# darnstrom/LinearMPC.jl

Hardware: AMD Instinct MI355X
Metric: condensed-MPC QP solves/sec (batch 1e6 params), pendulum Nc=5 (higher is better)
Workload: dtype f64; 1 GPU; pendulum: inverted pendulum on cart, 4 states / 1 input, Np=50 Nc=5 (n=5 vars, 5 two-sided input bounds, theta=[x;r;u_prev] nth=7), 1000000 parameter points per GPU, cold start, first move u0 returned; batch_per_gpu=1000000, kernel=fast<5>|screen+lane<5>, batches_in_flight=3, rotating_batches=6

## Files before the change

### linearmpc.jl_amd/csrc/lmpc_fast_inst.hip

```cpp
#include <hip/hip_runtime.h>

#include <cstdio>
#include <cstdlib>
#include <vector>

#include "lmpc_internal.hpp"
#include "lmpc_fast_kernel.hpp"

namespace lmpc {

bool fast_covers(const lmpc_handle *h) {
    const HostPack &P = h->P;
    constexpr int kmax = LMPC_FAST_KMAX;
    return h->fastPath && !h->useWave && h->laneN >= 2 && h->laneN <= 5 && P.n == h->laneN && P.m == P.n && P.ms == P.m &&
           P.nth >= 1 && P.nth <= (h->laneN == 5 ? 8 : 16) && h->L.eq_mask == 0ull && h->L.imm_mask == 0ull && P.nsoft == 0 && !h->bnb &&
           h->S.iter_limit > kmax + 1 && h->S.cycle_tol >= kmax + 1;
}

template <int NTHMAX, int NT, int N, bool GATHER>
static int launch_fast_t(lmpc_handle *h, int64_t nprob, const double *theta, double *x, int32_t *flag, int32_t *iters,
                         uint64_t *active, hipStream_t st) {
    const int nstr = h->fastNstr >= 1 && h->fastNstr <= 4 ? h->fastNstr : 3;
    const long long ntiles = (nprob + 63) / 64;
    long long slots = (long long)h->numCU * LMPC_FAST_WAVES;
    long long Rl = (ntiles + slots - 1) / slots;
    if (Rl < 8) Rl = 8;
    if (h->fastTiles > 0) Rl = h->fastTiles;
    if (Rl > kFastMaxTiles) Rl = kFastMaxTiles;
    if (Rl > ntiles) Rl = ntiles > 0 ? ntiles : 1;
    const int R = (int)Rl;
    const unsigned grid = (unsigned)((ntiles + R - 1) / R);
    int D = GATHER ? 0 : (h->fastDyn >= 0 ? h->fastDyn : 0);
    if (R < 12 || nprob >= (int64_t)0x7fffff00 || D >= R) D = 0;
    const int Rs = R - D, Dcap = 3 * D, Rq = D ? Rs + Dcap + 1 : R;
    int dk = GATHER ? 0 : (h->fastDma >= 0 ? h->fastDma : (nstr <= 3 ? LMPC_FAST_DMA_DEPTH : 0));
    if (dk == 1 || dk > 3) dk = dk == 1 ? 0 : 3;
    if (nprob * (int64_t)NT * 8 < 16) dk = 0;
    if ((reinterpret_cast<uintptr_t>(theta) & 15u) != 0 || (fast_tile_bytes(NT) & 15u) != 0) dk = 0;
    const size_t lds = dk ? fast_lds_bytes_dma(N, Rq, NTHMAX, NT, nstr, dk) : fast_lds_bytes(N, Rq, NTHMAX);
    int32_t *ctrNow = nullptr, *ctrNext = nullptr;
    if (D) {
        if (!h->dFastCtr) {
            HIP_TRY(h, hipMalloc(&h->dFastCtr, sizeof(int32_t) * 2 * kFastCtrs * 32));
            HIP_TRY(h, hipMemsetAsync(h->dFastCtr, 0, sizeof(int32_t) * 2 * kFastCtrs * 32, st));
        }
        ctrNow = h->dFastCtr + (size_t)h->fastCtrSet * kFastCtrs * 32;
        ctrNext = h->dFastCtr + (size_t)(h->fastCtrSet ^ 1) * kFastCtrs * 32;
        h->fastCtrSet ^= 1;
    }
    auto kern = fast_kernel<NTHMAX, NT, N, GATHER>;
    if (lds > 48 * 1024)
        HIP_TRY(h, hipFuncSetAttribute((const void *)kern, hipFuncAttributeMaxDynamicSharedMemorySize, (int)lds));
    if (!h->dFastErr) {
#ifdef LMPC_FAST_TRACE
        const size_t eb = 64 + sizeof(long long) * 8 * 4 * 65536;
        HIP_TRY(h, hipMalloc(&h->dFastErr, eb));
        HIP_TRY(h, hipMemsetAsync(h->dFastErr, 0, eb, st));
#else
        int32_t *hp = nullptr;
        HIP_TRY(h, hipHostMalloc(reinterpret_cast<void **>(&hp), 64, hipHostMallocMapped));
        *hp = 0;
        h->hFastErr = hp;
        HIP_TRY(h, hipHostGetDevicePointer(reinterpret_cast<void **>(&h->dFastErr), hp, 0));
#endif
    }
    hipLaunchKernelGGL(kern, dim3(grid), dim3(256), lds, st, h->L, h->dC, theta, x, flag, iters,
                       active, (long long)nprob, Rq, nstr, h->dFastErr, h->fastSpinLimit > 0 ? h->fastSpinLimit - 1 : kFastSpinLimit,
                       dk, Rs, Dcap, ctrNow, ctrNext);
    HIP_TRY(h, hipGetLastError());
#ifdef LMPC_FAST_TRACE
    if (const char *f = std::getenv("LMPC_FAST_TRACE_FILE")) {
        std::vector<long long> tr((size_t)grid * 4 * 8);
        if (hipStreamSynchronize(st) == hipSuccess &&
            hipMemcpy(tr.data(), reinterpret_cast<char *>(h->dFastErr) + 64, sizeof(long long) * tr.size(), hipMemcpyDeviceToHost) == hipSuccess) {
            if (FILE *fp = std::fopen(f, "wb")) { std::fwrite(tr.data(), sizeof(long long), tr.size(), fp); std::fclose(fp); }
        }
    }
#endif
    return LMPC_OK;
}

template <int NTHMAX, int NT, int N>
static int launch_fast_multi_t(lmpc_handle *h, int nb, int64_t nprob, const double *const *theta, double *const *x,
                               int32_t *const *flag, hipStream_t st) {
    const int nstr = h->fastNstr >= 1 && h->fastNstr <= 4 ? h->fastNstr : 3;
    const long long ntiles = (nprob + 63) / 64;
    long long slots = (long long)h->numCU * LMPC_FAST_WAVES;
    long long Rl = (ntiles + slots - 1) / slots;
    if (Rl < 8) Rl = 8;
    if (h->fastTiles > 0) Rl = h->fastTiles;
    if (Rl > kFastMaxTiles) Rl = kFastMaxTiles;
    if (Rl > ntiles) Rl = ntiles > 0 ? ntiles : 1;
    const int R = (int)Rl;
    const unsigned grid = (unsigned)((ntiles + R - 1) / R);
    int dk = h->fastDma >= 0 ? h->fastDma : (nstr <= 3 ? LMPC_FAST_DMA_DEPTH : 0);
    if (dk == 1 || dk > 3) dk = dk == 1 ? 0 : 3;
    if (nprob * (int64_t)NT * 8 < 16 || (fast_tile_bytes(NT) & 15u) != 0) dk = 0;
    FastBatches B{};
    for (int b = 0; b < nb; b++) {
        B.theta[b] = theta[b]; B.x[b] = x[b]; B.flag[b] = flag[b];
        if ((reinterpret_cast<uintptr_t>(theta[b]) & 15u) != 0) dk = 0;
    }
    const size_t lds = dk ? fast_lds_bytes_dma(N, R, NTHMAX, NT, nstr, dk) : fast_lds_bytes(N, R, NTHMAX);
    auto kern = fast_kernel_multi<NTHMAX, NT, N>;
    if (lds > 48 * 1024)
        HIP_TRY(h, hipFuncSetAttribute((const void *)kern, hipFuncAttributeMaxDynamicSharedMemorySize, (int)lds));
    if (!h->dFastErr) {
        int32_t *hp = nullptr;
        HIP_TRY(h, hipHostMalloc(reinterpret_cast<void **>(&hp), 64, hipHostMallocMapped));
        *hp = 0;
        h->hFastErr = hp;
        HIP_TRY(h, hipHostGetDevicePointer(reinterpret_cast<void **>(&h->dFastErr), hp, 0));
    }
    hipLaunchKernelGGL(kern, dim3(grid, (unsigned)nb), dim3(256), lds, st, h->L, h->dC, B, (long long)nprob, R, nstr, h->dFastErr,
                       h->fastSpinLimit > 0 ? h->fastSpinLimit - 1 : kFastSpinLimit, dk);
    HIP_TRY(h, hipGetLastError());
    return LMPC_OK;
}

int launch_fast_multi(lmpc_handle *h, int nb, int64_t nprob, const double *const *theta, double *const *x, int32_t *const *flag,
                      hipStream_t st) {
    if (nb < 1 || nb > kFastMaxBatches) return LMPC_ERR_UNSUPPORTED;
#ifdef LMPC_FAST_TRACE
    return LMPC_ERR_UNSUPPORTED;
#else
#define LMPC_FM(NM, NT)                                                                                     \
    switch (h->laneN) {                                                                                     \
        case 2: return launch_fast_multi_t<NM, NT, 2>(h, nb, nprob, theta, x, flag, st);                    \
        case 3: return launch_fast_multi_t<NM, NT, 3>(h, nb, nprob, theta, x, flag, st);                    \
        case 4: return launch_fast_multi_t<NM, NT, 4>(h, nb, nprob, theta, x, flag, st);                    \
        case 5: if constexpr (NT <= 8) return launch_fast_multi_t<NM, NT, 5>(h, nb, nprob, theta, x, flag, st); break; \
        default: break;                                                                                     \
    }                                                                                                       \
    break;
    switch (h->P.nth) {
#ifdef LMPC_FAST_ONLY_PENDULUM
        case 7: if (h->laneN == 5) return launch_fast_multi_t<8, 7, 5>(h, nb, nprob, theta, x, flag, st); break;
#else
        case 1: LMPC_FM(8, 1)   case 2: LMPC_FM(8, 2)   case 3: LMPC_FM(8, 3)   case 4: LMPC_FM(8, 4)
        case 5: LMPC_FM(8, 5)   case 6: LMPC_FM(8, 6)   case 7: LMPC_FM(8, 7)   case 8: LMPC_FM(8, 8)
        case 9: LMPC_FM(16, 9)  case 10: LMPC_FM(16, 10) case 11: LMPC_FM(16, 11) case 12: LMPC_FM(16, 12)
        case 13: LMPC_FM(16, 13) case 14: LMPC_FM(16, 14) case 15: LMPC_FM(16, 15) case 16: LMPC_FM(16, 16)
#endif
        default: break;
    }
#undef LMPC_FM
    return LMPC_ERR_UNSUPPORTED;
#endif
}

int check_fast_err(lmpc_handle *h) {
    if (!h->hFastErr) return LMPC_OK;
    const int32_t e = *h->hFastErr;
    if (e == 0) return LMPC_OK;
    *h->hFastErr = 0;
    return fail(h, LMPC_ERR_HIP, "lmpc: the one-launch kernel gave up a bounded wait (code " + std::to_string(e) +
                                 ") in an earlier call on this handle: problems it had queued keep exit flag -8 "
                                 "(LMPC_EXIT_UNFINISHED), their x is not a solution");
}

void fast_preload(lmpc_handle *h) {
    hipFuncAttributes fa;
    (void)hipFuncGetAttributes(&fa, (const void *)fast_kernel<8, 7, 5, false>);
    if (h && !h->dFastCtr && hipMalloc(&h->dFastCtr, sizeof(int32_t) * 2 * kFastCtrs * 32) == hipSuccess)
        (void)hipMemset(h->dFastCtr, 0, sizeof(int32_t) * 2 * kFastCtrs * 32);
#ifndef LMPC_FAST_TRACE
    if (h && !h->dFastErr) {
        int32_t *hp = nullptr;
        if (hipHostMalloc(reinterpret_cast<void **>(&hp), 64, hipHostMallocMapped) == hipSuccess) {
            *hp = 0;
            if (hipHostGetDevicePointer(reinterpret_cast<void **>(&h->dFastErr), hp, 0) == hipSuccess) h->hFastErr = hp;
            else { (void)hipHostFree(hp); h->dFastErr = nullptr; }
        }
    }
#endif
    (void)hipGetLastError();
}

int launch_fast(lmpc_handle *h, int64_t nprob, const double *theta, double *x, int32_t *flag, int32_t *iters,
                uint64_t *active, hipStream_t st) {
    const bool gather = h->L.gat.state != nullptr;
#define LMPC_FN(NM, NT)                                                                                               \
    switch (h->laneN) {                                                                                               \
        case 2: return gather ? launch_fast_t<NM, NT, 2, true>(h, nprob, theta, x, flag, iters, active, st) : launch_fast_t<NM, NT, 2, false>(h, nprob, theta, x, flag, iters, active, st);    \
        case 3: return gather ? launch_fast_t<NM, NT, 3, true>(h, nprob, theta, x, flag, iters, active, st) : launch_fast_t<NM, NT, 3, false>(h, nprob, theta, x, flag, iters, active, st);    \
        case 4: return gather ? launch_fast_t<NM, NT, 4, true>(h, nprob, theta, x, flag, iters, active, st) : launch_fast_t<NM, NT, 4, false>(h, nprob, theta, x, flag, iters, active, st);    \
        case 5: if constexpr (NT <= 8) return gather ? launch_fast_t<NM, NT, 5, true>(h, nprob, theta, x, flag, iters, active, st) : launch_fast_t<NM, NT, 5, false>(h, nprob, theta, x, flag, iters, active, st); break; \
        default: break;                                                                                               \
    }                                                                                                                 \
    break;
    switch (h->P.nth) {
#ifdef LMPC_FAST_ONLY_PENDULUM
        case 7: if (h->laneN == 5) return gather ? launch_fast_t<8, 7, 5, true>(h, nprob, theta, x, flag, iters, active, st) : launch_fast_t<8, 7, 5, false>(h, nprob, theta, x, flag, iters, active, st); break;
#else
        case 1: LMPC_FN(8, 1)   case 2: LMPC_FN(8, 2)   case 3: LMPC_FN(8, 3)   case 4: LMPC_FN(8, 4)
        case 5: LMPC_FN(8, 5)   case 6: LMPC_FN(8, 6)   case 7: LMPC_FN(8, 7)   case 8: LMPC_FN(8, 8)
        case 9: LMPC_FN(16, 9)  case 10: LMPC_FN(16, 10) case 11: LMPC_FN(16, 11) case 12: LMPC_FN(16, 12)
        case 13: LMPC_FN(16, 13) case 14: LMPC_FN(16, 14) case 15: LMPC_FN(16, 15) case 16: LMPC_FN(16, 16)
#endif
        default: break;
    }
#undef LMPC_FN
    return fail(h, LMPC_ERR_UNSUPPORTED, "lmpc: no fast-kernel instantiation");
}

}
```

### linearmpc.jl_amd/csrc/lmpc_fast_kernel.hpp

```cpp
#pragma once

#include <hip/hip_runtime.h>
#include <stdint.h>

#include "lmpc_lane_kernel.hpp"
#include "lmpc_tiers.hpp"

namespace lmpc {

#ifndef LMPC_FAST_WAVES
#define LMPC_FAST_WAVES 3
#endif
constexpr int kFastSpinLimit = 1 << 22;
constexpr int kFastCtrs = 16;
constexpr int kFastMaxTiles = 96;
#ifndef LMPC_FAST_AHEAD
#define LMPC_FAST_AHEAD 1
#endif
constexpr int kFastAhead = LMPC_FAST_AHEAD;

#ifndef LMPC_FAST_DMA_POLICY
#define LMPC_FAST_DMA_POLICY " nt"
#endif
__device__ __forceinline__ void fast_dma16(const void *gsrc, unsigned lds_dst) {
    unsigned keep;
    asm volatile("s_mov_b32 %0, m0\n\ts_mov_b32 m0, %2\n\ts_nop 0\n\tglobal_load_lds_dwordx4 %1, off" LMPC_FAST_DMA_POLICY
                 "\n\ts_mov_b32 m0, %0"
                 : "=&s"(keep) : "v"(gsrc), "s"(lds_dst) : "memory");
}
#ifndef LMPC_FAST_DMA_DEPTH
#define LMPC_FAST_DMA_DEPTH 2
#endif
__host__ __device__ constexpr size_t fast_tile_bytes(int NT) { return (size_t)64 * NT * sizeof(double); }

__device__ __forceinline__ int lds_load(const int *p) {
    return __hip_atomic_load(p, __ATOMIC_RELAXED, __HIP_MEMORY_SCOPE_WORKGROUP);
}

__host__ __device__ constexpr int fast_scr_doubles(int N, int NTHMAX) { return (N * NTHMAX + 2 * N + NTHMAX + 1 + 1) & ~1; }
#ifndef LMPC_FAST_PAY
#define LMPC_FAST_PAY 256
#endif
constexpr int kFastPay = LMPC_FAST_PAY;
__host__ __device__ constexpr size_t fast_lds_bytes(int N, int R, int NTHMAX) {
    return sizeof(double) * (size_t)(((N * N + N * (N + 1) / 2 + 2 * N + 1) & ~1) + 4 * N * 64 + fast_scr_doubles(N, NTHMAX) +
                                     (size_t)kFastPay * (N + 1)) +
           sizeof(int32_t) * ((size_t)R * 64 + 4);
}
__host__ __device__ constexpr size_t fast_lds_bytes_dma(int N, int R, int NTHMAX, int NT, int nstr, int dk) {
    return fast_lds_bytes(N, R, NTHMAX) + (size_t)dk * nstr * fast_tile_bytes(NT);
}

template <int NTHMAX, int NT, int N, bool GATHER = false>
__device__ __forceinline__ void fast_body(
    const PackLayout &P, const double *__restrict__ C, const double *__restrict__ theta,
    double *__restrict__ X, int32_t *__restrict__ exitflag, int32_t *__restrict__ iters,
    uint64_t *__restrict__ active, long long nprob, int R, int nstr, int32_t *__restrict__ errflag, int spinLimit,
    int dk, int Rs, int Dcap, int32_t *__restrict__ tctr, int32_t *__restrict__ tctr_next) {
    constexpr int KMAX = LMPC_FAST_KMAX < N ? LMPC_FAST_KMAX : N;
    constexpr int nconst = N * N + N * (N + 1) / 2 + 2 * N;
    extern __shared__ __align__(16) double lds[];
    double *sconst = lds;
    double *sBall = sconst + ((nconst + 1) & ~1);
    double *sScr = sBall + 4 * N * 64;
    double *sPay = sScr + fast_scr_doubles(N, NTHMAX);
    int32_t *ring = reinterpret_cast<int32_t *>(sPay + (size_t)kFastPay * (N + 1));
    int *ctrl = reinterpret_cast<int *>(ring + R * 64);
    const int tid = threadIdx.x, lane = tid & 63;
    const int wv = __builtin_amdgcn_readfirstlane(tid >> 6);
    const int nth = P.nth;
    for (int i = tid; i < nconst; i += 256) sconst[i] = C[P.oM + i];
    for (int i = tid; i < N * NTHMAX; i += 256) sScr[i] = C[P.oDthP + i];
    if (tid < 2 * N) sScr[N * NTHMAX + tid] = C[P.oBnd + tid];
    if (tid < NTHMAX) sScr[N * NTHMAX + 2 * N + tid] = C[P.oXthP + tid];
    if (tid == 0) sScr[N * NTHMAX + 2 * N + NTHMAX] = C[P.ox0];
    for (int i = tid; i < R * 64; i += 256) ring[i] = -1;
    if (tid < 4) ctrl[tid] = 0;
    __syncthreads();
    const double *sM = sconst, *sG = sM + N * N, *sdu = sG + N * (N + 1) / 2, *sdl = sdu + N;
    double *sB = sBall + wv * N * 64;
    const double ntol = -P.primal_tol;
    const long long ntiles = (nprob + 63) / 64;
#ifdef LMPC_FAST_TRACE
    long long *trc = reinterpret_cast<long long *>(errflag + 16) + ((long long)blockIdx.x * 4 + wv) * 8;
    int npass = 0;
#define LMPC_TRC(i) do { if (lane == 0) trc[i] = (long long)wall_clock64(); } while (0)
#else
#define LMPC_TRC(i) do { } while (0)
#endif
    LMPC_TRC(0);
    const bool dyn = tctr != nullptr;
    const long long nstat = dyn ? ((long long)gridDim.x * Rs < ntiles ? (long long)gridDim.x * Rs : ntiles) : ntiles;
    if (dyn && blockIdx.x == 0 && tid < kFastCtrs) tctr_next[tid * 32] = 0;
    const long long t0 = (long long)blockIdx.x * (dyn ? Rs : R);
    const long long t1 = t0 + (dyn ? Rs : R) < nstat ? t0 + (dyn ? Rs : R) : nstat;
    const long long base0 = dyn ? 0 : t0 * 64;

    auto load_record = [&](long long pid, double *dst) {
        const long long pc = pid < nprob ? pid : nprob - 1;
        if constexpr (GATHER) {
            const GatherArgs &Ga = P.gat;
            const int o1 = Ga.nx, o2 = o1 + Ga.nr, o3 = o2 + Ga.nd, o4 = o3 + Ga.nup;
#pragma unroll
            for (int t = 0; t < NT; t++) {
                double v = 0.0;
                if (t < o1) v = Ga.state[pc * Ga.nx + t];
                else if (t < o2) { if (Ga.reference) v = Ga.reference[pc * Ga.nr + (t - o1)]; }
                else if (t < o3) { if (Ga.disturbance) v = Ga.disturbance[pc * Ga.nd + (t - o2)]; }
                else if (t < o4) { if (Ga.control) v = Ga.control[pc * Ga.ncontrol + (t - o3)]; }
                else { if (Ga.parameter) v = Ga.parameter[pc * Ga.np + (t - o4)]; }
                dst[t] = v;
            }
        } else {
            const double *src = theta + pc * nth;
#pragma unroll
            for (int t = 0; t < NT; t++) dst[t] = src[t];
        }
    };
    auto write_x = [&](long long pid, const double (&th)[NT], const double (&u)[N], bool with_u) {
        const double *xk = C + P.oXthP;
        for (int k = 0; k < P.nout; k++, xk += NTHMAX) {
            double sh = C[P.ox0 + k];
#pragma unroll
            for (int t = 0; t < NT; t++) sh = __builtin_fma(xk[t], th[t], sh);
            double xs = 0.0;
            if (with_u) {
#pragma unroll
                for (int c = 0; c < N; c++) xs = __builtin_fma(C[P.oRout + k * N + c], u[c], xs);
            }
            X[pid * P.nout + k] = xs + sh;
        }
    };

    const int role = (wv + (int)(blockIdx.x & 3)) & 3;
    if (role < nstr) {
        double buf[kFastAhead][NT];
        auto process = [&](long long tile, const double (&th)[NT], bool live) {
            const long long pid = tile * 64 + lane;
            const bool valid = live && pid < nprob;
            typedef const double __attribute__((address_space(3))) *lds_cdp;
            unsigned scr_off = (unsigned)(size_t)(lds_cdp)sScr;
            asm volatile("" : "+v"(scr_off));
            const lds_cdp scr = (lds_cdp)(size_t)scr_off;
            bool hard = false;
            typedef double v2d __attribute__((ext_vector_type(2)));
            typedef const v2d __attribute__((address_space(3))) *lds_c2p;
            const lds_c2p c2 = (lds_c2p)(size_t)scr_off;
            static_assert(NTHMAX % 2 == 0, "rows of pairs");
            double bq[N];
#pragma unroll
            for (int j = 0; j < N; j++) {
                double row[NTHMAX];
#pragma unroll
                for (int q = 0; q < (NT + 1) / 2; q++) {
                    const v2d v = c2[j * (NTHMAX / 2) + q];
                    row[2 * q] = v.x; row[2 * q + 1] = v.y;
                }
                double acc = 0.0;
#pragma unroll
                for (int t = 0; t < NT; t++) acc = __builtin_fma(row[t], th[t], acc);
                bq[j] = acc;
                const v2d bb = c2[N * (NTHMAX / 2) + j];
                const double vu = (bb.x + acc) - 0.0;
                const double vl = -((bb.y + acc) - 0.0);
                hard = hard | (vu < ntol) | (vl < ntol);
            }
            hard = hard & valid;
            double sh = scr[N * NTHMAX + 2 * N + NTHMAX];
            {
                double row[NTHMAX];
#pragma unroll
                for (int q = 0; q < (NT + 1) / 2; q++) {
                    const v2d v = c2[(N * NTHMAX + 2 * N) / 2 + q];
                    row[2 * q] = v.x; row[2 * q + 1] = v.y;
                }
#pragma unroll
                for (int t = 0; t < NT; t++) sh = __builtin_fma(row[t], th[t], sh);
            }
            const unsigned long long mask = __ballot(hard);
#ifdef LMPC_FAST_NT_STORES
            if (valid) __builtin_nontemporal_store(hard ? EXIT_UNFINISHED : EXIT_OPTIMAL, &exitflag[pid]);
#else
            if (valid) exitflag[pid] = hard ? EXIT_UNFINISHED : EXIT_OPTIMAL;
#endif
            if (mask != 0ull) {
                int base = 0;
                if (lane == 0) base = __hip_atomic_fetch_add(&ctrl[0], __popcll(mask), __ATOMIC_RELAXED, __HIP_MEMORY_SCOPE_WORKGROUP);
                base = __shfl(base, 0);
                if (hard) {
                    const int pos = base + __popcll(mask & ((1ull << lane) - 1ull));
                    if (pos < kFastPay) {
                        double *pay = sPay + pos * (N + 1);
#pragma unroll
                        for (int j = 0; j < N; j++) pay[j] = bq[j];
                        pay[N] = sh;
                    }
                    __hip_atomic_store(&ring[pos], (int32_t)(pid - base0), __ATOMIC_RELEASE, __HIP_MEMORY_SCOPE_WORKGROUP);
                }
            }
            if (valid && !hard) {
                if (P.nout == 1) {
#ifdef LMPC_FAST_NT_STORES
                    __builtin_nontemporal_store(0.0 + sh, &X[pid]);
#else
                    X[pid] = 0.0 + sh;
#endif
                } else {
                    double u0[N];
#pragma unroll
                    for (int c = 0; c < N; c++) u0[c] = 0.0;
                    write_x(pid, th, u0, false);
                }
                if (iters) iters[pid] = 1;
                if (active) active[pid * P.words] = 0ull;
            }
        };
#ifdef LMPC_FAST_CONTIG
        const long long per = (R + nstr - 1) / nstr;
        const long long s0 = t0 + role * per, s1 = s0 + per < t1 ? s0 + per : t1;
        for (long long base = s0; base < s1; base += kFastAhead) {
#pragma unroll
            for (int d = 0; d < kFastAhead; d++) {
                const long long tl = base + d;
                load_record((tl < s1 ? tl : base) * 64 + lane, buf[d]);
            }
#pragma unroll
            for (int d = 0; d < kFastAhead; d++) {
                const long long tl = base + d;
                process(tl < s1 ? tl : base, buf[d], tl < s1);
            }
        }
#elif defined(LMPC_FAST_PP)
        {
            double bufB[NT];
            long long tile = t0 + role;
            if (tile < t1) {
                load_record(tile * 64 + lane, buf[0]);
                for (;;) {
                    long long nxt = tile + nstr < t1 ? tile + nstr : tile;
                    load_record(nxt * 64 + lane, bufB);
                    process(tile, buf[0], true);
                    if (tile + nstr >= t1) break;
                    tile += nstr;
                    nxt = tile + nstr < t1 ? tile + nstr : tile;
                    load_record(nxt * 64 + lane, buf[0]);
                    process(tile, bufB, true);
                    if (tile + nstr >= t1) break;
                    tile += nstr;
                }
            }
        }
#else
        if (!GATHER && dk >= 2) {
            constexpr unsigned TB = (unsigned)fast_tile_bytes(NT);
            constexpr int PIECES = (int)((TB + 1023) / 1024);
            constexpr unsigned LASTB = TB - (PIECES - 1) * 1024u;
            typedef const double __attribute__((address_space(3))) *lds_cdp;
            char *dring = reinterpret_cast<char *>(ctrl + 4) + (size_t)role * dk * TB;
            const unsigned dbase = (unsigned)(size_t)(lds_cdp) reinterpret_cast<double *>(dring);
            const char *tbytes = reinterpret_cast<const char *>(theta);
            const long long tfull = nprob / 64;
            const long long te = t1 < tfull ? t1 : tfull;
            auto issue = [&](long long tile, int slot) {
                const char *src = tbytes + tile * (long long)TB + lane * 16;
#pragma unroll
                for (int p = 0; p < PIECES; p++) {
                    const unsigned dst = __builtin_amdgcn_readfirstlane(dbase + (unsigned)slot * TB + (unsigned)p * 1024u);
                    if (p + 1 < PIECES || LASTB == 1024u || lane * 16 < (int)LASTB) fast_dma16(src + p * 1024, dst);
                }
            };
            int cc = (int)((blockIdx.x * (unsigned)nstr + (unsigned)role) & (kFastCtrs - 1));
            auto take = [&]() -> long long {
                int t = -1;
                if (lane == 0) {
                    if (__hip_atomic_fetch_add(&ctrl[3], 1, __ATOMIC_RELAXED, __HIP_MEMORY_SCOPE_WORKGROUP) < Dcap)
                        t = atomicAdd(&tctr[cc * 32], 1);
                }
                t = __builtin_amdgcn_readfirstlane(t);
                const long long tile = nstat + (long long)t * kFastCtrs + cc;
                return (t >= 0 && tile < ntiles) ? tile : -1;
            };
            if (dk == 2) {
                long long sidx = t0 + role, tk = -1;
                bool drew = false;
                auto take_full = [&]() -> long long { const long long t = take(); return t < tfull ? t : -1; };
                if (dyn && sidx >= te) tk = take_full();
                auto peek = [&]() -> long long { return sidx < te ? sidx : (dyn ? tk : -1); };
                auto advance = [&]() {
                    drew = false;
                    if (sidx < te) { sidx += nstr; if (dyn && sidx >= te) { tk = take_full(); drew = true; } }
                    else if (dyn && tk >= 0) { tk = take_full(); drew = true; }
                };
                long long cur = peek();
                int sc = 0;
                if (cur >= 0) { issue(cur, 0); advance(); }
                while (cur >= 0) {
                    const long long nxt = peek();
                    const bool nd = nxt >= 0;
                    if (nd) { issue(nxt, sc ^ 1); advance(); } else drew = false;
                    if (nd && drew) asm volatile("s_waitcnt vmcnt(%0)" :: "n"(PIECES + 1) : "memory");
                    else if (nd) asm volatile("s_waitcnt vmcnt(%0)" :: "n"(PIECES) : "memory");
                    else asm volatile("s_waitcnt vmcnt(0)" ::: "memory");
                    const double *rec = reinterpret_cast<const double *>(dring + (size_t)sc * TB) + lane * NT;
#pragma unroll
                    for (int t = 0; t < NT; t++) buf[0][t] = rec[t];
                    process(cur, buf[0], true);
                    cur = nxt;
                    sc ^= 1;
                }
                const long long part = dyn ? ((blockIdx.x == 0 && role == 0 && tfull < ntiles) ? tfull : -1)
                                           : ((sidx < t1 && sidx == tfull) ? tfull : -1);
                if (part >= 0) {
                    load_record(part * 64 + lane, buf[0]);
                    process(part, buf[0], true);
                }
            } else {
            const long long first = t0 + role;
            long long ahead = first;
            int sa = 0;
            for (int d = 0; d < dk - 1 && ahead < te; d++, ahead += nstr) { issue(ahead, sa); sa = sa + 1 == dk ? 0 : sa + 1; }
            int sc = 0;
            long long tile = first;
            for (; tile < te; tile += nstr) {
                if (ahead < te) { issue(ahead, sa); sa = sa + 1 == dk ? 0 : sa + 1; ahead += nstr; }
                const long long younger = (ahead - tile) / nstr - 1;
                if (younger >= 2) asm volatile("s_waitcnt vmcnt(%0)" :: "n"(2 * PIECES) : "memory");
                else if (younger == 1) asm volatile("s_waitcnt vmcnt(%0)" :: "n"(PIECES) : "memory");
                else asm volatile("s_waitcnt vmcnt(0)" ::: "memory");
                const double *rec = reinterpret_cast<const double *>(dring + (size_t)sc * TB) + lane * NT;
#pragma unroll
                for (int t = 0; t < NT; t++) buf[0][t] = rec[t];
                sc = sc + 1 == dk ? 0 : sc + 1;
                process(tile, buf[0], true);
            }
            if (tile < t1) {
                load_record(tile * 64 + lane, buf[0]);
                process(tile, buf[0], true);
            }
            if (dyn) {
                long long tl = take();
                while (tl >= 0) {
                    load_record(tl * 64 + lane, buf[0]);
                    const long long nx = take();
                    process(tl, buf[0], true);
                    tl = nx;
                }
            }
            }
        } else
        for (long long base = t0 + role; base < t1; base += (long long)kFastAhead * nstr) {
#pragma unroll
            for (int d = 0; d < kFastAhead; d++) {
                const long long tl = base + (long long)d * nstr;
                load_record((tl < t1 ? tl : base) * 64 + lane, buf[d]);
            }
#pragma unroll
            for (int d = 0; d < kFastAhead; d++) {
                const long long tl = base + (long long)d * nstr;
                process(tl < t1 ? tl : base, buf[d], tl < t1);
            }
        }
#endif
        if (dyn && !(!GATHER && dk >= 2)) {
            int cc = (int)((blockIdx.x * (unsigned)nstr + (unsigned)role) & (kFastCtrs - 1));
            auto take = [&]() -> long long {
                int t = -1;
                if (lane == 0) {
                    if (__hip_atomic_fetch_add(&ctrl[3], 1, __ATOMIC_RELAXED, __HIP_MEMORY_SCOPE_WORKGROUP) < Dcap)
                        t = atomicAdd(&tctr[cc * 32], 1);
                }
                t = __builtin_amdgcn_readfirstlane(t);
                const long long tile = nstat + (long long)t * kFastCtrs + cc;
                return (t >= 0 && tile < ntiles) ? tile : -1;
            };
            long long tile = take();
            while (tile >= 0) {
                load_record(tile * 64 + lane, buf[0]);
                const long long nxt = take();
                process(tile, buf[0], true);
                tile = nxt;
            }
        }
        if (lane == 0) __hip_atomic_fetch_add(&ctrl[2], 1, __ATOMIC_RELEASE, __HIP_MEMORY_SCOPE_WORKGROUP);
        LMPC_TRC(1);
    }

    int spins = 0;
    for (;;) {
        int start = 0, n = 0;
        if (lane == 0) {
            for (;;) {
                const int d = __hip_atomic_load(&ctrl[2], __ATOMIC_ACQUIRE, __HIP_MEMORY_SCOPE_WORKGROUP);
                const int w = lds_load(&ctrl[0]);
                int r = lds_load(&ctrl[1]);
                const int avail = w - r;
                if (avail >= 64 || (d >= nstr && avail > 0)) {
                    const int take = avail < 64 ? avail : 64;
                    if (__hip_atomic_compare_exchange_strong(&ctrl[1], &r, r + take, __ATOMIC_RELAXED, __ATOMIC_RELAXED,
                                                             __HIP_MEMORY_SCOPE_WORKGROUP)) { start = r; n = take; break; }
                } else if (d >= nstr) {
                    n = -1;
                    break;
                } else {
                    __builtin_amdgcn_s_sleep(8);
                }
                if (++spins > spinLimit) { n = -2; break; }
            }
        }
        start = __builtin_amdgcn_readfirstlane(start);
        n = __builtin_amdgcn_readfirstlane(n);
        if (n == -2 && lane == 0 && errflag) __hip_atomic_store(errflag, 1, __ATOMIC_RELAXED, __HIP_MEMORY_SCOPE_SYSTEM);
        if (n < 0) break;
#ifdef LMPC_FAST_TRACE
        if (npass < 2) LMPC_TRC(2 + npass);
        npass++;
#endif
#ifdef LMPC_FAST_PRIO
        __builtin_amdgcn_s_setprio(LMPC_FAST_PRIO);
#endif
        const bool mine = lane < n;
        int rel = -1;
        if (mine) {
            int sp = 0;
            while ((rel = __hip_atomic_load(&ring[start + lane], __ATOMIC_ACQUIRE, __HIP_MEMORY_SCOPE_WORKGROUP)) < 0) {
                if (++sp > spinLimit) break;
            }
        }
        if (__any(mine && rel < 0)) {
            if (lane == 0 && errflag) __hip_atomic_store(errflag, 2, __ATOMIC_RELAXED, __HIP_MEMORY_SCOPE_SYSTEM);
            break;
        }
        const long long pid = mine ? base0 + rel : base0;
        double b[N], u[N];
        double sh0 = C[P.ox0];
        const bool handed = start + lane < kFastPay;
#pragma unroll
        for (int j = 0; j < N; j++) b[j] = 0.0;
        if (handed) {
            const double *pay = sPay + (start + (mine ? lane : 0)) * (N + 1);
#pragma unroll
            for (int j = 0; j < N; j++) b[j] = pay[j];
            sh0 = pay[N];
        }
        if (__any(mine && !handed)) {
            double th0[NT];
            load_record(pid, th0);
            const double *dj = C + P.oDthP;
            double sh1 = C[P.ox0];
#pragma unroll
            for (int j = 0; j < N; j++) {
                double acc = 0.0;
#pragma unroll
                for (int t = 0; t < NT; t++) acc = __builtin_fma(dj[j * NTHMAX + t], th0[t], acc);
                b[j] = handed ? b[j] : acc;
            }
            const double *xk = C + P.oXthP;
#pragma unroll
            for (int t = 0; t < NT; t++) sh1 = __builtin_fma(xk[t], th0[t], sh1);
            sh0 = handed ? sh0 : sh1;
        }
#ifdef LMPC_FAST_TRACE
        if (npass == 1) { if (lane == 0) trc[4] = (long long)(b[0] != 12345.678 ? wall_clock64() : 0); }
#endif
        int iter = 1, nact = 0, wrow[KMAX], flag = EXIT_ITERLIMIT;
        bool wlow[KMAX];
        unsigned long long act = 0ull, low = 0ull;
        const int res = fast_tiers<N, KMAX>(P, sM, sG, sdu, sdl, mine, b, u, iter, wrow, wlow, nact);
        bool solved = res == EXIT_OPTIMAL;
#ifdef LMPC_FAST_TRACE
        if (npass == 1) { if (lane == 0) trc[5] = (long long)(res != 77 ? wall_clock64() : 0); }
#endif
        if (solved) {
            flag = EXIT_OPTIMAL;
#pragma unroll
            for (int i = 0; i < KMAX; i++)
                if (i < nact) { act |= 1ull << wrow[i]; if (wlow[i]) low |= 1ull << wrow[i]; }
        }
#ifndef LMPC_FAST_NO_FALLBACK
        if (mine && !solved) {
#pragma unroll
            for (int j = 0; j < N; j++) sB[j * 64 + lane] = b[j];
            LaneState<N, N> s;
            s.init();
            lane_loop<N, N, N, false>(P, C, sM, sG, sdu, sdl, sB, 64, lane, pid, nullptr, s);
#pragma unroll
            for (int c = 0; c < N; c++) u[c] = s.u[c];
            flag = s.flag; iter = s.iter; act = s.act; low = s.low;
        }
#endif
        if (mine) {
            if (P.nout == 1) {
                double xs = 0.0;
#pragma unroll
                for (int c = 0; c < N; c++) xs = __builtin_fma(C[P.oRout + c], u[c], xs);
                X[pid] = xs + sh0;
            } else {
                double th[NT];
                load_record(pid, th);
                write_x(pid, th, u, true);
            }
            exitflag[pid] = flag;
            if (iters) iters[pid] = iter;
            if (active) active[pid * P.words] = (act & ~low) | ((act & low) << N);
        }
#ifdef LMPC_FAST_PRIO
        __builtin_amdgcn_s_setprio(0);
#endif
    }
    LMPC_TRC(6);
#ifdef LMPC_FAST_TRACE
    if (lane == 0) trc[7] = (long long)npass | ((long long)(unsigned)__builtin_amdgcn_s_getreg((31 << 11) | 4) << 16) |
                            ((long long)((unsigned)__builtin_amdgcn_s_getreg((31 << 11) | 20) & 0xffu) << 48);
#endif
#undef LMPC_TRC
}

template <int NTHMAX, int NT, int N, bool GATHER = false>
__global__ __launch_bounds__(256, LMPC_FAST_WAVES) void fast_kernel(
    const PackLayout P, const double *__restrict__ C, const double *__restrict__ theta,
    double *__restrict__ X, int32_t *__restrict__ exitflag, int32_t *__restrict__ iters,
    uint64_t *__restrict__ active, long long nprob, int R, int nstr, int32_t *__restrict__ errflag, int spinLimit,
    int dk, int Rs, int Dcap, int32_t *__restrict__ tctr, int32_t *__restrict__ tctr_next) {
    fast_body<NTHMAX, NT, N, GATHER>(P, C, theta, X, exitflag, iters, active, nprob, R, nstr, errflag, spinLimit, dk, Rs, Dcap, tctr,
                                     tctr_next);
}

constexpr int kFastMaxBatches = 8;
struct FastBatches {
    const double *theta[kFastMaxBatches];
    double *x[kFastMaxBatches];
    int32_t *flag[kFastMaxBatches];
};
template <int NTHMAX, int NT, int N>
__global__ __launch_bounds__(256, LMPC_FAST_WAVES) void fast_kernel_multi(
    const PackLayout P, const double *__restrict__ C, const FastBatches B, long long nprob, int R, int nstr,
    int32_t *__restrict__ errflag, int spinLimit, int dk) {
    const int b = blockIdx.y;
    fast_body<NTHMAX, NT, N, false>(P, C, B.theta[b], B.x[b], B.flag[b], nullptr, nullptr, nprob, R, nstr, errflag, spinLimit, dk, R, 0,
                                    nullptr, nullptr);
}

}
```

Baseline: 62.50 billion solves/s.

## Outline fast-path fallback solver and drop per-wave LDS scratch

Moves the rare fallback active-set solve into a noinline device function that keeps its shift vector in registers instead of a per-wave LDS slab. This removes 4*N*64 doubles of LDS per block and may lower register pressure in the hot fast-tier path. LMPC_FAST_WAVES goes from 3 to 4, which likely sets the launch bound or occupancy target, while grid sizing stays pinned at 3 waves through a new constant. It also deletes the unused CONTIG and PP loop variants. The cost is a function call with argument marshalling whenever the fallback runs, plus possible register spills in the outlined code.

Result: faster. 66.03 billion solves/s (median of 6 runs) (+5.6%).

```diff
diff --git a/linearmpc.jl_amd/csrc/lmpc_fast_inst.hip b/linearmpc.jl_amd/csrc/lmpc_fast_inst.hip
--- a/linearmpc.jl_amd/csrc/lmpc_fast_inst.hip
+++ b/linearmpc.jl_amd/csrc/lmpc_fast_inst.hip
@@ -22,7 +22,7 @@
                          uint64_t *active, hipStream_t st) {
     const int nstr = h->fastNstr >= 1 && h->fastNstr <= 4 ? h->fastNstr : 3;
     const long long ntiles = (nprob + 63) / 64;
-    long long slots = (long long)h->numCU * LMPC_FAST_WAVES;
+    long long slots = (long long)h->numCU * kFastGridWaves;
     long long Rl = (ntiles + slots - 1) / slots;
     if (Rl < 8) Rl = 8;
     if (h->fastTiles > 0) Rl = h->fastTiles;
@@ -85,7 +85,7 @@
                                int32_t *const *flag, hipStream_t st) {
     const int nstr = h->fastNstr >= 1 && h->fastNstr <= 4 ? h->fastNstr : 3;
     const long long ntiles = (nprob + 63) / 64;
-    long long slots = (long long)h->numCU * LMPC_FAST_WAVES;
+    long long slots = (long long)h->numCU * kFastGridWaves;
     long long Rl = (ntiles + slots - 1) / slots;
     if (Rl < 8) Rl = 8;
     if (h->fastTiles > 0) Rl = h->fastTiles;
diff --git a/linearmpc.jl_amd/csrc/lmpc_fast_kernel.hpp b/linearmpc.jl_amd/csrc/lmpc_fast_kernel.hpp
--- a/linearmpc.jl_amd/csrc/lmpc_fast_kernel.hpp
+++ b/linearmpc.jl_amd/csrc/lmpc_fast_kernel.hpp
@@ -9,8 +9,9 @@
 namespace lmpc {
 
 #ifndef LMPC_FAST_WAVES
-#define LMPC_FAST_WAVES 3
-#endif
+#define LMPC_FAST_WAVES 4
+#endif
+constexpr int kFastGridWaves = 3;
 constexpr int kFastSpinLimit = 1 << 22;
 constexpr int kFastCtrs = 16;
 constexpr int kFastMaxTiles = 96;
@@ -43,12 +44,47 @@
 #endif
 constexpr int kFastPay = LMPC_FAST_PAY;
 __host__ __device__ constexpr size_t fast_lds_bytes(int N, int R, int NTHMAX) {
-    return sizeof(double) * (size_t)(((N * N + N * (N + 1) / 2 + 2 * N + 1) & ~1) + 4 * N * 64 + fast_scr_doubles(N, NTHMAX) +
+    return sizeof(double) * (size_t)(((N * N + N * (N + 1) / 2 + 2 * N + 1) & ~1) + fast_scr_doubles(N, NTHMAX) +
                                      (size_t)kFastPay * (N + 1)) +
            sizeof(int32_t) * ((size_t)R * 64 + 4);
 }
 __host__ __device__ constexpr size_t fast_lds_bytes_dma(int N, int R, int NTHMAX, int NT, int nstr, int dk) {
     return fast_lds_bytes(N, R, NTHMAX) + (size_t)dk * nstr * fast_tile_bytes(NT);
+}
+
+template <int N> struct FastShifts { double b[N]; };
+template <int N> struct FastFallback { double u[N]; unsigned long long act, low; int flag, iter; };
+struct FastLoopArgs {
+    unsigned long long imm_mask, eq_mask;
+    double primal_tol, dual_tol, zero_tol, progress_tol, fval_bound;
+    int n, m, words, oM, odu, odl, cycle_tol, iter_limit;
+};
+__device__ __forceinline__ FastLoopArgs fast_loop_args(const PackLayout &P) {
+    return FastLoopArgs{P.imm_mask, P.eq_mask, P.primal_tol, P.dual_tol, P.zero_tol, P.progress_tol, P.fval_bound,
+                        P.n, P.m, P.words, P.oM, P.odu, P.odl, P.cycle_tol, P.iter_limit};
+}
+template <int N>
+__device__ __attribute__((noinline)) FastFallback<N> fast_fallback(const FastLoopArgs A, const double *__restrict__ C,
+                                                                    const FastShifts<N> sh, const long long pid) {
+    PackLayout P{};
+    P.imm_mask = A.imm_mask; P.eq_mask = A.eq_mask;
+    P.primal_tol = A.primal_tol; P.dual_tol = A.dual_tol; P.zero_tol = A.zero_tol; P.progress_tol = A.progress_tol;
+    P.fval_bound = A.fval_bound;
+    P.n = A.n; P.m = A.m; P.words = A.words; P.oM = A.oM; P.odu = A.odu; P.odl = A.odl;
+    P.cycle_tol = A.cycle_tol; P.iter_limit = A.iter_limit;
+    extern __shared__ __align__(16) double lds[];
+    const double *sM = lds, *sG = sM + N * N, *sdu = sG + N * (N + 1) / 2, *sdl = sdu + N;
+    double sB[N];
+#pragma unroll
+    for (int j = 0; j < N; j++) sB[j] = sh.b[j];
+    LaneState<N, N> s;
+    s.init();
+    lane_loop<N, N, N, false>(P, C, sM, sG, sdu, sdl, sB, 1, 0, pid, nullptr, s);
+    FastFallback<N> r;
+#pragma unroll
+    for (int c = 0; c < N; c++) r.u[c] = s.u[c];
+    r.act = s.act; r.low = s.low; r.flag = s.flag; r.iter = s.iter;
+    return r;
 }
 
 template <int NTHMAX, int NT, int N, bool GATHER = false>
@@ -61,8 +97,7 @@
     constexpr int nconst = N * N + N * (N + 1) / 2 + 2 * N;
     extern __shared__ __align__(16) double lds[];
     double *sconst = lds;
-    double *sBall = sconst + ((nconst + 1) & ~1);
-    double *sScr = sBall + 4 * N * 64;
+    double *sScr = sconst + ((nconst + 1) & ~1);
     double *sPay = sScr + fast_scr_doubles(N, NTHMAX);
     int32_t *ring = reinterpret_cast<int32_t *>(sPay + (size_t)kFastPay * (N + 1));
     int *ctrl = reinterpret_cast<int *>(ring + R * 64);
@@ -78,7 +113,6 @@
     if (tid < 4) ctrl[tid] = 0;
     __syncthreads();
     const double *sM = sconst, *sG = sM + N * N, *sdu = sG + N * (N + 1) / 2, *sdl = sdu + N;
-    double *sB = sBall + wv * N * 64;
     const double ntol = -P.primal_tol;
     const long long ntiles = (nprob + 63) / 64;
 #ifdef LMPC_FAST_TRACE
@@ -215,42 +249,6 @@
                 if (active) active[pid * P.words] = 0ull;
             }
         };
-#ifdef LMPC_FAST_CONTIG
-        const long long per = (R + nstr - 1) / nstr;
-        const long long s0 = t0 + role * per, s1 = s0 + per < t1 ? s0 + per : t1;
-        for (long long base = s0; base < s1; base += kFastAhead) {
-#pragma unroll
-            for (int d = 0; d < kFastAhead; d++) {
-                const long long tl = base + d;
-                load_record((tl < s1 ? tl : base) * 64 + lane, buf[d]);
-            }
-#pragma unroll
-            for (int d = 0; d < kFastAhead; d++) {
-                const long long tl = base + d;
-                process(tl < s1 ? tl : base, buf[d], tl < s1);
-            }
-        }
-#elif defined(LMPC_FAST_PP)
-        {
-            double bufB[NT];
-            long long tile = t0 + role;
-            if (tile < t1) {
-                load_record(tile * 64 + lane, buf[0]);
-                for (;;) {
-                    long long nxt = tile + nstr < t1 ? tile + nstr : tile;
-                    load_record(nxt * 64 + lane, bufB);
-                    process(tile, buf[0], true);
-                    if (tile + nstr >= t1) break;
-                    tile += nstr;
-                    nxt = tile + nstr < t1 ? tile + nstr : tile;
-                    load_record(nxt * 64 + lane, buf[0]);
-                    process(tile, bufB, true);
-                    if (tile + nstr >= t1) break;
-                    tile += nstr;
-                }
-            }
-        }
-#else
         if (!GATHER && dk >= 2) {
             constexpr unsigned TB = (unsigned)fast_tile_bytes(NT);
             constexpr int PIECES = (int)((TB + 1023) / 1024);
@@ -360,7 +358,6 @@
                 process(tl < t1 ? tl : base, buf[d], tl < t1);
             }
         }
-#endif
         if (dyn && !(!GATHER && dk >= 2)) {
             int cc = (int)((blockIdx.x * (unsigned)nstr + (unsigned)role) & (kFastCtrs - 1));
             auto take = [&]() -> long long {
@@ -478,14 +475,13 @@
         }
 #ifndef LMPC_FAST_NO_FALLBACK
         if (mine && !solved) {
-#pragma unroll
-            for (int j = 0; j < N; j++) sB[j * 64 + lane] = b[j];
-            LaneState<N, N> s;
-            s.init();
-            lane_loop<N, N, N, false>(P, C, sM, sG, sdu, sdl, sB, 64, lane, pid, nullptr, s);
-#pragma unroll
-            for (int c = 0; c < N; c++) u[c] = s.u[c];
-            flag = s.flag; iter = s.iter; act = s.act; low = s.low;
+            FastShifts<N> bs;
+#pragma unroll
+            for (int j = 0; j < N; j++) bs.b[j] = b[j];
+            const FastFallback<N> r = fast_fallback<N>(fast_loop_args(P), C, bs, pid);
+#pragma unroll
+            for (int c = 0; c < N; c++) u[c] = r.u[c];
+            flag = r.flag; iter = r.iter; act = r.act; low = r.low;
         }
 #endif
         if (mine) {
```
